# mlefkir/Pioran.jl

Measured on AMD Instinct MI355X. Metric: logpdf evals/sec (batched) at N=1e4, J=20; max |Δlogℒ| vs reference, higher is better.
Workload: dtype f64; 1 GPU; N=10000 irregular series, SHO-20 (J=20 celerite terms, R=40 active rows), batch=4096 draws per GPU, shared (c,d), per-draw mu/nu; inputs HBM-resident; N=10000, J=20, R_active=40, batch_per_gpu=4096, global_batch=4096, kernel_config=tile, parallelism=batch-sharded x1, all-gather of logL

## Files before the change

pioran.jl_amd/csrc/celerite_tile.hip:

```cpp
#include "common.h"
#include "window_common.h"

#ifndef PIORAN_TSTAMP
#define PIORAN_TSTAMP(i) __builtin_amdgcn_sched_barrier(0)
#define PIORAN_TSTAMP_DECL
#define PIORAN_TSTAMP_FLUSH
#endif
#ifndef PIORAN_ASTAMP2
#define PIORAN_ASTAMP2(i) __builtin_amdgcn_sched_barrier(0)
#define PIORAN_ASTAMP2_DECL
#define PIORAN_ASTAMP2_FLUSH
#endif

namespace {

#ifndef PIORAN_TILE_FWD_NOWAIT
#define PIORAN_TILE_FWD_NOWAIT 1
#endif
#if PIORAN_TILE_FWD_NOWAIT
#define PIORAN_TILE_FWD_ORDER() asm volatile("" ::: "memory")
#else
#define PIORAN_TILE_FWD_ORDER() asm volatile("s_waitcnt lgkmcnt(0)" ::: "memory")
#endif
#ifndef PIORAN_TILE_ADJ_RAGFIX
#define PIORAN_TILE_ADJ_RAGFIX 1
#endif
#ifndef PIORAN_TILE_RAGFIX4
#define PIORAN_TILE_RAGFIX4 1
#endif
#ifndef PIORAN_TILE_QUADALL
#define PIORAN_TILE_QUADALL 1
#endif
#ifndef PIORAN_TILE_RAGFIX
#define PIORAN_TILE_RAGFIX 1
#endif
#ifndef PIORAN_TILE_YSFIX
#define PIORAN_TILE_YSFIX 1
#endif
#ifndef PIORAN_TILE_BIG_VHA
#define PIORAN_TILE_BIG_VHA 1
#endif
#ifndef PIORAN_TILE_BIG_CKP
#define PIORAN_TILE_BIG_CKP 1
#endif
#ifndef PIORAN_TILE_VHA
#define PIORAN_TILE_VHA 1
#endif
constexpr int kTileMaxTerms = 64;
constexpr int kTileWaves = 4;
#define PIORAN_LDS_ORDER() asm volatile("" ::: "memory")
template <int NB, bool CD = false>
constexpr int tile_adj_waves() { return NB <= 3 ? 4 : (CD ? 2 : 3); }

typedef unsigned int tile_u32x2 __attribute__((ext_vector_type(2)));
__device__ __forceinline__ double tile_bload(__amdgpu_buffer_rsrc_t rs, int voff, int soff)
{
    const tile_u32x2 v = __builtin_amdgcn_raw_buffer_load_b64(rs, voff, soff, 0);
    return __hiloint2double((int)v.y, (int)v.x);
}

template <int NB>
struct TileWave {
    double scr[16 * 18];
    double2 albe[16 * NB];
    double ck[16 * NB + 16];
    double ys[16];
    double up[NB > 1 ? NB * (NB - 1) / 2 : 1][16 * 18];
};

constexpr int kPairWin = 5;
template <int JQ>
__global__ void __launch_bounds__(256) tile_pairs_mfma_kernel(const ScanParams p, const double* __restrict__ btab, int64_t rsb, int64_t tsp, double* __restrict__ out)
{
    const int J = p.J;
    const int64_t NW = (p.N + KW - 1) / KW;
    const int lane = threadIdx.x & 63, w = threadIdx.x >> 6, li = lane & 15, lk = lane >> 4;
    const int64_t b0 = ((int64_t)blockIdx.y * 4 + w) * 16;
    if (b0 >= p.B) return;
    const int64_t draw = b0 + li < p.B ? b0 + li : p.B - 1;
    double aop[JQ], bop[JQ];
    int toff[JQ];
#pragma unroll
    for (int q = 0; q < JQ; ++q) {
        const int t = 4 * q + lk;
        aop[q] = t < J ? p.A[draw * J + t] : 0.0;
        bop[q] = t < J ? p.Bc[draw * J + t] : 0.0;
        toff[q] = (t < J ? t : J - 1) * 128 + 4 * (li & 3) + (li >> 2);
    }
    const bool live = b0 + li < p.B;
    double* orow = out + (b0 + li) * NW * 128 + 4 * lk;
    const int64_t k0 = (int64_t)blockIdx.x * kPairWin, k1 = k0 + kPairWin < NW ? k0 + kPairWin : NW;
    for (int64_t k = k0; k < k1; ++k) {
        const double2* E = reinterpret_cast<const double2*>(btab + k * rsb + tsp);
#pragma unroll 2
        for (int pt = 0; pt < 8; ++pt) {
            double2 e[JQ];
#pragma unroll
            for (int q = 0; q < JQ; ++q) e[q] = E[toff[q] + 16 * pt];
            d4 acc = {0.0, 0.0, 0.0, 0.0};
#pragma unroll
            for (int q = 0; q < JQ; ++q) {
                acc = __builtin_amdgcn_mfma_f64_16x16x4f64(e[q].x, aop[q], acc, 0, 0, 0);
                acc = __builtin_amdgcn_mfma_f64_16x16x4f64(e[q].y, bop[q], acc, 0, 0, 0);
            }
            if (live) *reinterpret_cast<d4*>(orow + k * 128 + 16 * pt) = acc;
        }
    }
}

template <typename... Args>
static inline bool launch_pairs_mfma(const ScanParams& p, hipStream_t stream, Args... args)
{
    const int64_t NW = (p.N + KW - 1) / KW;
    if ((p.B + 63) / 64 > 65535 || p.J > kTileMaxTerms) return false;
    const dim3 gr((unsigned)((NW + kPairWin - 1) / kPairWin), (unsigned)((p.B + 63) / 64));
    const int jq = (p.J + 3) / 4;
    if (jq <= 5) hipLaunchKernelGGL(tile_pairs_mfma_kernel<5>, gr, dim3(256), 0, stream, p, args...);
    else if (jq <= 10) hipLaunchKernelGGL(tile_pairs_mfma_kernel<10>, gr, dim3(256), 0, stream, p, args...);
    else if (jq <= 16) hipLaunchKernelGGL(tile_pairs_mfma_kernel<16>, gr, dim3(256), 0, stream, p, args...);
    else return false;
    return true;
}

template <int NB, int KL = 4, bool ST = false>
__global__ void __launch_bounds__(64 * kTileWaves, NB <= 4 ? 2 : 1) celerite_tile_kernel(const ScanParams p, const double* __restrict__ btab,
                                                                                          const double* __restrict__ pairs)
// ... 29 lines not shown
            const int rm = p.rowmap[r];
            const int term = rm & 0xfffff;
            a = Ab_[term];
            bb = ((rm >> 30) & 1) ? -Bb_[term] : Bb_[term];
        }
        sw.albe[r] = double2{a, bb};
    }
    constexpr int NU = NB * (NB - 1) / 2;
    for (int i = lane; i < (NU > 0 ? NU : 1) * 16 * 18; i += 64) (&sw.up[0][0])[i] = 0.0;
    asm volatile("s_waitcnt lgkmcnt(0)" ::: "memory");

    constexpr int NT = NB * (NB + 1) / 2;
    auto tix = [](int I, int Jc) constexpr { return I * (I + 1) / 2 + Jc; };
    auto uix = [](int I, int Jc) constexpr { return I * (I - 1) / 2 + Jc; };
    d4 T[NT];
#pragma unroll
    for (int i = 0; i < NT; ++i) T[i] = d4{0.0, 0.0, 0.0, 0.0};
    double Uf[NB][4];

    double cvn[4], cxn[4];
    auto live_k = [](int I, int ks) constexpr { return I < NB - 1 || ks < KL; };
    auto fetch_u = [&](int64_t k, int I) __attribute__((always_inline)) {
        const int so = (int)k * rsb8;
#pragma unroll
        for (int ks = 0; ks < 4; ++ks) {
            if (!live_k(I, ks)) continue;
            cvn[ks] = tile_bload(rs_tab, lane8, so + (I * 4 + ks) * 512);
            cxn[ks] = tile_bload(rs_tab, lane8, so + (NB * 256 + (I * 4 + ks) * 64) * 8);
        }
    };
    auto form_u = [&](int I) __attribute__((always_inline)) {
        if (I == NB - 1 && KL == 0) return;
        double2 cf[4];
#pragma unroll
        for (int ks = 0; ks < 4; ++ks)
            if (live_k(I, ks)) cf[ks] = sw.albe[16 * I + 4 * ks + q];
        asm volatile("s_waitcnt lgkmcnt(0)" ::: "memory");
#pragma unroll
        for (int ks = 0; ks < 4; ++ks)
            if (live_k(I, ks)) Uf[I][ks] = fma(cf[ks].x, cvn[ks], cf[ks].y * cxn[ks]);
    };
    constexpr int NCK = (16 * NB + 16 + 63) / 64;
    double ckpre[NCK];
    auto fetch_ck = [&](int64_t k) __attribute__((always_inline)) {
        const int so = (int)k * rsb8 + 3 * NB * 256 * 8;
#pragma unroll
        for (int i = 0; i < NCK; ++i) ckpre[i] = tile_bload(rs_tab, lane8, so + 512 * i);
    };
    int pidx[4];
#pragma unroll
    for (int g = 0; g < 4; ++g) {
        const int r = 4 * g + q, hi = r > c16 ? r : c16, lo = r > c16 ? c16 : r;
        pidx[g] = 8 * (r == c16 ? 127 : hi * (hi - 1) / 2 + lo);
    }
    const int gd = (c16 - q) >> 2;
    const bool on_diag = ((c16 - q) & 3) == 0;
    double apre[4];
    auto fetch_A = [&](int64_t k) __attribute__((always_inline)) {
#pragma unroll
        for (int g = 0; g < 4; ++g) apre[g] = tile_bload(rs_pw, pidx[g], (int)k * 1024);
    };
    const bool has_series = p.Y != nullptr;
    double ypre = 0.0, spre = 0.0;
    auto fetch_series = [&](int64_t k) __attribute__((always_inline)) {
        if (has_series) {
            int64_t n = k * KW + c16;
            n = n < N ? n : N - 1;
            ypre = p.Y[b * N + n];
            spre = p.S2[b * N + n];
        }
    };
    fetch_A(0);
    fetch_ck(0);
    fetch_series(0);
#pragma unroll
    for (int I = 0; I < NB; ++I) {
        fetch_u(0, I);
        form_u(I);
    }
    double mu_sel[NB];
#pragma unroll
    for (int Jc = 0; Jc < NB; ++Jc) mu_sel[Jc] = (Jc == Jy && c16 == ry) ? mu : 0.0;
    const int64_t k_ragged = (N % KW) ? NW - 1 : NW;
    double quad = 0.0;
#if PIORAN_TILE_QUADALL
    double quadb[NB];
#pragma unroll
    for (int I = 0; I < NB; ++I) quadb[I] = 0.0;
#endif
    double Pm = 1.0;
    int Pe = 0;
    bool nonpd = false;

    PIORAN_TSTAMP_DECL
    for (int64_t k = 0; k < NW; ++k) {
        PIORAN_TSTAMP(0);
        const int wso = (int)k * rsb8;
        const bool more = k + 1 < NW;
#pragma unroll
        for (int i = 0; i < NCK; ++i)
            if (lane + 64 * i < 16 * NB + 16) sw.ck[lane + 64 * i] = ckpre[i];
        if (has_series) {
            asm volatile("s_waitcnt lgkmcnt(0)" ::: "memory");
            if (lane < 16) { sw.ys[lane] = ypre; sw.ck[16 * NB + lane] = spre; }
        }
        if (more) { fetch_ck(k + 1); fetch_series(k + 1); }
        if constexpr (ST) {
            d4* gtk = reinterpret_cast<d4*>(p.gw + ((b * NW + k) * NT) * 256);
#pragma unroll
            for (int i = 0; i < NT; ++i) gtk[i * 64 + lane] = T[i];
        }
        constexpr bool VHA = PIORAN_TILE_VHA && (NB <= 3 || (PIORAN_TILE_BIG_VHA && NB >= 5));
        [[maybe_unused]] double vha[VHA ? NB : 1][4];
        if constexpr (VHA) {
#pragma unroll
            for (int I = 0; I < NB; ++I)
#pragma unroll
                for (int g = 0; g < 4; ++g) vha[I][g] = tile_bload(rs_tab, lane8, wso + (2 * NB * 256 + (I * 4 + g) * 64) * 8);
#if PIORAN_TILE_RAGFIX
            if (k == k_ragged) {
#pragma unroll
                for (int I = 0; I < NB; ++I)
#pragma unroll
                    for (int g = 0; g < 4; ++g)
                        if (k * KW + 4 * g + q >= N) vha[I][g] = mu_sel[I];
            }
#endif
        }
        d4 x[NB];
#pragma unroll
        for (int Jc = 0; Jc < NB; ++Jc) {
            d4 acc = {0.0, 0.0, 0.0, 0.0};
#pragma unroll
            for (int I = 0; I < Jc; ++I) {
                double bt[4];
#pragma unroll
                for (int ks = 0; ks < 4; ++ks) bt[ks] = sw.up[uix(Jc, I)][c16 * 18 + 4 * ks + q];
#pragma unroll
                for (int ks = 0; ks < 4; ++ks) acc = __builtin_amdgcn_mfma_f64_16x16x4f64(Uf[I][ks], bt[ks], acc, 0, 0, 0);
            }
#pragma unroll
            for (int I = Jc; I < NB; ++I)
#pragma unroll
                for (int ks = 0; ks < 4; ++ks)
                    if (live_k(I, ks)) acc = __builtin_amdgcn_mfma_f64_16x16x4f64(Uf[I][ks], T[tix(I, Jc)][ks], acc, 0, 0, 0);
            x[Jc] = acc;
        }
        PIORAN_TSTAMP(1);
        d4 G = {0.0, 0.0, 0.0, 0.0};
        double vh[4];
        if constexpr (!VHA) {
#pragma unroll
            for (int g = 0; g < 4; ++g) vh[g] = tile_bload(rs_tab, lane8, wso + (2 * NB * 256 + g * 64) * 8);
        }
        double ysv[4] = {0.0, 0.0, 0.0, 0.0};
        if (has_series) {
#pragma unroll
            for (int g = 0; g < 4; ++g) ysv[g] = sw.ys[4 * g + q];
        }
#pragma unroll
        for (int Jc = 0; Jc < NB; ++Jc) {
            const bool gk = Jc < NB - 1 || KL > 0;
            if (gk) {
#pragma unroll
                for (int g = 0; g < 4; ++g) sw.scr[(4 * g + q) * 18 + c16] = x[Jc][g];
            }
            PIORAN_TILE_FWD_ORDER();
            double mb[4];
#pragma unroll
            for (int ks = 0; ks < 4; ++ks)
                if (live_k(Jc, ks)) mb[ks] = sw.scr[c16 * 18 + 4 * ks + q];
            const double ckc = sw.ck[16 * Jc + c16];
            asm volatile("s_waitcnt lgkmcnt(0)" ::: "memory");
#pragma unroll
            for (int ks = 0; ks < 4; ++ks)
                if (live_k(Jc, ks)) G = __builtin_amdgcn_mfma_f64_16x16x4f64(Uf[Jc][ks], mb[ks], G, 0, 0, 0);
#pragma unroll
            for (int g = 0; g < 4; ++g) {
                double v;
                if constexpr (VHA) v = vha[Jc][g]; else v = vh[g];
#if !PIORAN_TILE_YSFIX
                if (has_series && Jc == Jy && c16 == ry) v = ysv[g];
#endif
                v -= mu_sel[Jc];
#if PIORAN_TILE_RAGFIX && !PIORAN_TILE_RAGFIX4
                if constexpr (!VHA)
#endif
#if !PIORAN_TILE_RAGFIX4
                if (k == k_ragged && k * KW + 4 * g + q >= N) v = 0.0;
#endif
                x[Jc][g] = fma(-ckc, x[Jc][g], v);
                asm volatile("" : "+v"(x[Jc][g]));
            }
            if constexpr (!VHA) {
                if (Jc + 1 < NB) {
#pragma unroll
                    for (int g = 0; g < 4; ++g) vh[g] = tile_bload(rs_tab, lane8, wso + (2 * NB * 256 + ((Jc + 1) * 4 + g) * 64) * 8);
                }
            }
            __builtin_amdgcn_sched_barrier(0);
        }
#if PIORAN_TILE_RAGFIX4
        if constexpr (!VHA) {
            if (k == k_ragged) {
#pragma unroll
                for (int Jc = 0; Jc < NB; ++Jc)
#pragma unroll
                    for (int g = 0; g < 4; ++g) {
                        const double vt = tile_bload(rs_tab, lane8, wso + (2 * NB * 256 + (Jc * 4 + g) * 64) * 8);
                        if (k * KW + 4 * g + q >= N) x[Jc][g] -= vt - mu_sel[Jc];
                    }
            }
        }
#endif
#if PIORAN_TILE_YSFIX
        if (has_series) {
            static_for<0, NB>([&](auto Jcc) __attribute__((always_inline)) {
                constexpr int Jc = decltype(Jcc)::value;
                if (Jc == Jy) {
#pragma unroll
                    for (int g = 0; g < 4; ++g) {
                        double vt;
                        if constexpr (VHA) vt = vha[Jc][g]; else vt = tile_bload(rs_tab, lane8, wso + (2 * NB * 256 + (Jc * 4 + g) * 64) * 8);
                        const bool pad = k == k_ragged && k * KW + 4 * g + q >= N;
                        if (c16 == ry && !pad) x[Jc][g] += ysv[g] - vt;
                    }
                }
            });
        }
#endif
        PIORAN_TSTAMP(2);
        PIORAN_TSTAMP(3);
        {
            const double s2n = sw.ck[16 * NB + c16];
            const double dg = k * KW + c16 < N ? suma + (has_nu ? nu * s2n : s2n) : 1.0;
#pragma unroll
            for (int g = 0; g < 4; ++g) sw.scr[(4 * g + q) * 16 + c16] = ((on_diag && g == gd) ? dg : apre[g]) - G[g];
        }
        if (k + 1 < NW) fetch_A(k + 1);
        PIORAN_TILE_FWD_ORDER();
        double m[16];
#pragma unroll
        for (int j = 0; j < 16; ++j) m[j] = sw.scr[j * 16 + c16];
        asm volatile("s_waitcnt lgkmcnt(0)" ::: "memory");
        PIORAN_TSTAMP(4);
        __builtin_amdgcn_s_setprio(2);
        double mult = ldl_first_mult(m, c16);
        static_for<0, 16>([&](auto Pc) __attribute__((always_inline)) { ldl_step<decltype(Pc)::value>(m, mult, c16); });
        __builtin_amdgcn_s_setprio(0);
        PIORAN_TSTAMP(5);
        if (q == 0) {
            double2* dst = reinterpret_cast<double2*>(sw.scr + c16 * 18);
#pragma unroll
            for (int j = 0; j < 16; j += 2) dst[j / 2] = double2{m[j], m[j + 1]};
        }
        PIORAN_TILE_FWD_ORDER();
        double li[4], idv[4];
#pragma unroll
        for (int ks = 0; ks < 4; ++ks) {
            const int kk = 4 * ks + q;
            const double lv = sw.scr[kk * 18 + c16];
            idv[ks] = recip_f64(sw.scr[kk * 18 + kk]);
            li[ks] = kk < c16 ? lv * idv[ks] : (kk == c16 ? 1.0 : 0.0);
        }
        {
            const double dj = sw.scr[c16 * 18 + c16];
            nonpd |= !(dj > 0.0);
            Pm *= (k == 0 && c16 == 0) ? dj : fabs(dj);
            int ex;
            Pm = frexp(Pm, &ex);
            Pe += ex;
        }
        asm volatile("s_waitcnt lgkmcnt(0)" ::: "memory");
        PIORAN_TSTAMP(6);
        if (more) fetch_u(k + 1, 0);
        __builtin_amdgcn_sched_barrier(0);
        d4 yt[NB];
#pragma unroll
        for (int Jc = 0; Jc < NB; ++Jc) {
            d4 a = {0.0, 0.0, 0.0, 0.0};
#pragma unroll
            for (int ks = 0; ks < 4; ++ks) a = __builtin_amdgcn_mfma_f64_16x16x4f64(li[ks], x[Jc][ks], a, 0, 0, 0);
            yt[Jc] = a;
        }
        PIORAN_TSTAMP(7);
        constexpr bool CKP = NB <= 3 || (PIORAN_TILE_BIG_CKP && NB >= 5);
        [[maybe_unused]] double ckrow[CKP ? NB : 1][4], ckcol[CKP ? NB : 1];
        if constexpr (CKP) {
#pragma unroll
            for (int I = 0; I < NB; ++I) {
#pragma unroll
                for (int g = 0; g < 4; ++g) ckrow[I][g] = sw.ck[16 * I + 4 * g + q];
                ckcol[I] = sw.ck[16 * I + c16];
            }
        }
        auto ck_row = [&](int I, int g) __attribute__((always_inline)) -> double { if constexpr (CKP) return ckrow[I][g]; else return sw.ck[16 * I + 4 * g + q]; };
#pragma unroll
        for (int Jc = 0; Jc < NB; ++Jc) {
            if (more) {
                form_u(Jc);
                if (Jc + 1 < NB) fetch_u(k + 1, Jc + 1);
            }
            double ysc[4];
            double ckc;
            if constexpr (CKP) ckc = ckcol[Jc]; else ckc = sw.ck[16 * Jc + c16];
#pragma unroll
            for (int g = 0; g < 4; ++g) {
                ysc[g] = yt[Jc][g] * idv[g];
#if PIORAN_TILE_QUADALL
                quadb[Jc] = fma(yt[Jc][g], ysc[g], quadb[Jc]);
#else
                if (Jc == Jy) quad = fma(yt[Jc][g], ysc[g], quad);
#endif
            }
#pragma unroll
            for (int I = Jc; I < NB; ++I) {
#pragma unroll
                for (int g = 0; g < 4; ++g) T[tix(I, Jc)][g] *= ck_row(I, g) * ckc;
#pragma unroll
                for (int ks = 0; ks < 4; ++ks) T[tix(I, Jc)] = __builtin_amdgcn_mfma_f64_16x16x4f64(yt[I][ks], ysc[ks], T[tix(I, Jc)], 0, 0, 0);
                if (Jc < I) {
#pragma unroll
                    for (int g = 0; g < 4; ++g) sw.up[uix(I, Jc)][(4 * g + q) * 18 + c16] = T[tix(I, Jc)][g];
                }
            }
            __builtin_amdgcn_sched_barrier(0);
        }
        PIORAN_TSTAMP(8);
        PIORAN_TILE_FWD_ORDER();
    }

    PIORAN_TSTAMP_FLUSH
    asm volatile("s_waitcnt lgkmcnt(0)" ::: "memory");
#if PIORAN_TILE_QUADALL
#pragma unroll
    for (int I = 0; I < NB; ++I)
        if (I == Jy) quad = quadb[I];
// ... 1010 lines not shown
```

pioran.jl_amd/csrc/ldl_steps.inc:

```
template <int P> __device__ __forceinline__ void ldl_step_fused(double (&m)[16], double& mult, int c16);
template <> __device__ __forceinline__ void ldl_step_fused<0>(double (&m)[16], double& mult, int c16)
{
    double dn, r0, e, t0, pq, mn;
    asm volatile("v_fmac_f64_dpp %[m1], %[m1], %[t] row_newbcast:0 row_mask:0xf bank_mask:0xf\n\t"
                 "s_nop 1\n\tv_mov_b64_dpp %[dn], %[m1] row_newbcast:1 row_mask:0xf bank_mask:0xf\n\t"
                 "v_rcp_f64 %[r0], %[dn]\n\t"
                 "v_fmac_f64_dpp %[m2], %[m2], %[t] row_newbcast:0 row_mask:0xf bank_mask:0xf\n\t"
                 "v_fmac_f64_dpp %[m3], %[m3], %[t] row_newbcast:0 row_mask:0xf bank_mask:0xf\n\t"
                 "v_fmac_f64_dpp %[m4], %[m4], %[t] row_newbcast:0 row_mask:0xf bank_mask:0xf\n\t"
                 "v_fmac_f64_dpp %[m5], %[m5], %[t] row_newbcast:0 row_mask:0xf bank_mask:0xf\n\t"
                 "v_fma_f64 %[e], -%[r0], %[dn], 1.0\n\tv_mul_f64 %[t0], -%[m1], %[r0]\n\t"
                 "v_fmac_f64_dpp %[m6], %[m6], %[t] row_newbcast:0 row_mask:0xf bank_mask:0xf\n\t"
                 "v_fmac_f64_dpp %[m7], %[m7], %[t] row_newbcast:0 row_mask:0xf bank_mask:0xf\n\t"
                 "v_fmac_f64_dpp %[m8], %[m8], %[t] row_newbcast:0 row_mask:0xf bank_mask:0xf\n\t"
                 "v_fmac_f64_dpp %[m9], %[m9], %[t] row_newbcast:0 row_mask:0xf bank_mask:0xf\n\t"
                 "v_fma_f64 %[pq], %[e], %[e], %[e]\n\t"
                 "v_fmac_f64_dpp %[m10], %[m10], %[t] row_newbcast:0 row_mask:0xf bank_mask:0xf\n\t"
                 "v_fmac_f64_dpp %[m11], %[m11], %[t] row_newbcast:0 row_mask:0xf bank_mask:0xf\n\t"
                 "v_fmac_f64_dpp %[m12], %[m12], %[t] row_newbcast:0 row_mask:0xf bank_mask:0xf\n\t"
                 "v_fmac_f64_dpp %[m13], %[m13], %[t] row_newbcast:0 row_mask:0xf bank_mask:0xf\n\t"
                 "v_fmac_f64_dpp %[m14], %[m14], %[t] row_newbcast:0 row_mask:0xf bank_mask:0xf\n\t"
                 "v_fmac_f64_dpp %[m15], %[m15], %[t] row_newbcast:0 row_mask:0xf bank_mask:0xf\n\t"
                 "v_fma_f64 %[mn], %[t0], %[pq], %[t0]"
                 : [m1] "+v"(m[1]), [m2] "+v"(m[2]), [m3] "+v"(m[3]), [m4] "+v"(m[4]), [m5] "+v"(m[5]), [m6] "+v"(m[6]), [m7] "+v"(m[7]), [m8] "+v"(m[8]), [m9] "+v"(m[9]), [m10] "+v"(m[10]), [m11] "+v"(m[11]), [m12] "+v"(m[12]), [m13] "+v"(m[13]), [m14] "+v"(m[14]), [m15] "+v"(m[15]), [dn] "=&v"(dn), [r0] "=&v"(r0), [e] "=&v"(e), [t0] "=&v"(t0), [pq] "=&v"(pq), [mn] "=&v"(mn)
// ... 195 lines not shown
                 "v_fma_f64 %[pq], %[e], %[e], %[e]\n\t"
                 "v_fma_f64 %[mn], %[t0], %[pq], %[t0]"
                 : [m10] "+v"(m[10]), [m11] "+v"(m[11]), [m12] "+v"(m[12]), [m13] "+v"(m[13]), [m14] "+v"(m[14]), [m15] "+v"(m[15]), [dn] "=&v"(dn), [r0] "=&v"(r0), [e] "=&v"(e), [t0] "=&v"(t0), [pq] "=&v"(pq), [mn] "=&v"(mn)
                 : [t] "v"(mult));
    mult = c16 == 10 ? -2.0 : mn;
}
template <> __device__ __forceinline__ void ldl_step_fused<10>(double (&m)[16], double& mult, int c16)
{
    double dn, r0, e, t0, pq, mn;
    asm volatile("v_fmac_f64_dpp %[m11], %[m11], %[t] row_newbcast:10 row_mask:0xf bank_mask:0xf\n\t"
                 "s_nop 1\n\tv_mov_b64_dpp %[dn], %[m11] row_newbcast:11 row_mask:0xf bank_mask:0xf\n\t"
                 "v_rcp_f64 %[r0], %[dn]\n\t"
                 "v_fmac_f64_dpp %[m12], %[m12], %[t] row_newbcast:10 row_mask:0xf bank_mask:0xf\n\t"
                 "v_fmac_f64_dpp %[m13], %[m13], %[t] row_newbcast:10 row_mask:0xf bank_mask:0xf\n\t"
                 "v_fmac_f64_dpp %[m14], %[m14], %[t] row_newbcast:10 row_mask:0xf bank_mask:0xf\n\t"
                 "v_fmac_f64_dpp %[m15], %[m15], %[t] row_newbcast:10 row_mask:0xf bank_mask:0xf\n\t"
                 "v_fma_f64 %[e], -%[r0], %[dn], 1.0\n\tv_mul_f64 %[t0], -%[m11], %[r0]\n\t"
                 "v_fma_f64 %[pq], %[e], %[e], %[e]\n\t"
                 "v_fma_f64 %[mn], %[t0], %[pq], %[t0]"
                 : [m11] "+v"(m[11]), [m12] "+v"(m[12]), [m13] "+v"(m[13]), [m14] "+v"(m[14]), [m15] "+v"(m[15]), [dn] "=&v"(dn), [r0] "=&v"(r0), [e] "=&v"(e), [t0] "=&v"(t0), [pq] "=&v"(pq), [mn] "=&v"(mn)
                 : [t] "v"(mult));
    mult = c16 == 11 ? -2.0 : mn;
}
template <> __device__ __forceinline__ void ldl_step_fused<11>(double (&m)[16], double& mult, int c16)
{
    double dn, r0, e, t0, pq, mn;
    asm volatile("v_fmac_f64_dpp %[m12], %[m12], %[t] row_newbcast:11 row_mask:0xf bank_mask:0xf\n\t"
                 "s_nop 1\n\tv_mov_b64_dpp %[dn], %[m12] row_newbcast:12 row_mask:0xf bank_mask:0xf\n\t"
                 "v_rcp_f64 %[r0], %[dn]\n\t"
                 "v_fmac_f64_dpp %[m13], %[m13], %[t] row_newbcast:11 row_mask:0xf bank_mask:0xf\n\t"
                 "v_fmac_f64_dpp %[m14], %[m14], %[t] row_newbcast:11 row_mask:0xf bank_mask:0xf\n\t"
                 "v_fmac_f64_dpp %[m15], %[m15], %[t] row_newbcast:11 row_mask:0xf bank_mask:0xf\n\t"
                 "v_fma_f64 %[e], -%[r0], %[dn], 1.0\n\tv_mul_f64 %[t0], -%[m12], %[r0]\n\t"
                 "v_fma_f64 %[pq], %[e], %[e], %[e]\n\t"
                 "v_fma_f64 %[mn], %[t0], %[pq], %[t0]"
                 : [m12] "+v"(m[12]), [m13] "+v"(m[13]), [m14] "+v"(m[14]), [m15] "+v"(m[15]), [dn] "=&v"(dn), [r0] "=&v"(r0), [e] "=&v"(e), [t0] "=&v"(t0), [pq] "=&v"(pq), [mn] "=&v"(mn)
                 : [t] "v"(mult));
    mult = c16 == 12 ? -2.0 : mn;
}
template <> __device__ __forceinline__ void ldl_step_fused<12>(double (&m)[16], double& mult, int c16)
{
    double dn, r0, e, t0, pq, mn;
    asm volatile("v_fmac_f64_dpp %[m13], %[m13], %[t] row_newbcast:12 row_mask:0xf bank_mask:0xf\n\t"
                 "s_nop 1\n\tv_mov_b64_dpp %[dn], %[m13] row_newbcast:13 row_mask:0xf bank_mask:0xf\n\t"
                 "v_rcp_f64 %[r0], %[dn]\n\t"
                 "v_fmac_f64_dpp %[m14], %[m14], %[t] row_newbcast:12 row_mask:0xf bank_mask:0xf\n\t"
                 "v_fmac_f64_dpp %[m15], %[m15], %[t] row_newbcast:12 row_mask:0xf bank_mask:0xf\n\t"
                 "v_fma_f64 %[e], -%[r0], %[dn], 1.0\n\tv_mul_f64 %[t0], -%[m13], %[r0]\n\t"
                 "v_fma_f64 %[pq], %[e], %[e], %[e]\n\t"
                 "v_fma_f64 %[mn], %[t0], %[pq], %[t0]"
                 : [m13] "+v"(m[13]), [m14] "+v"(m[14]), [m15] "+v"(m[15]), [dn] "=&v"(dn), [r0] "=&v"(r0), [e] "=&v"(e), [t0] "=&v"(t0), [pq] "=&v"(pq), [mn] "=&v"(mn)
                 : [t] "v"(mult));
    mult = c16 == 13 ? -2.0 : mn;
}
template <> __device__ __forceinline__ void ldl_step_fused<13>(double (&m)[16], double& mult, int c16)
{
    double dn, r0, e, t0, pq, mn;
    asm volatile("v_fmac_f64_dpp %[m14], %[m14], %[t] row_newbcast:13 row_mask:0xf bank_mask:0xf\n\t"
                 "s_nop 1\n\tv_mov_b64_dpp %[dn], %[m14] row_newbcast:14 row_mask:0xf bank_mask:0xf\n\t"
                 "v_rcp_f64 %[r0], %[dn]\n\t"
                 "v_fmac_f64_dpp %[m15], %[m15], %[t] row_newbcast:13 row_mask:0xf bank_mask:0xf\n\t"
                 "v_fma_f64 %[e], -%[r0], %[dn], 1.0\n\tv_mul_f64 %[t0], -%[m14], %[r0]\n\t"
                 "v_fma_f64 %[pq], %[e], %[e], %[e]\n\t"
                 "v_fma_f64 %[mn], %[t0], %[pq], %[t0]"
                 : [m14] "+v"(m[14]), [m15] "+v"(m[15]), [dn] "=&v"(dn), [r0] "=&v"(r0), [e] "=&v"(e), [t0] "=&v"(t0), [pq] "=&v"(pq), [mn] "=&v"(mn)
                 : [t] "v"(mult));
    mult = c16 == 14 ? -2.0 : mn;
}
template <> __device__ __forceinline__ void ldl_step_fused<14>(double (&m)[16], double& mult, int c16)
{
    double dn, r0, e, t0, pq, mn;
    asm volatile("v_fmac_f64_dpp %[m15], %[m15], %[t] row_newbcast:14 row_mask:0xf bank_mask:0xf\n\t"
                 "s_nop 1\n\tv_mov_b64_dpp %[dn], %[m15] row_newbcast:15 row_mask:0xf bank_mask:0xf\n\t"
                 "v_rcp_f64 %[r0], %[dn]\n\t"
                 "s_nop 0\n\t"
                 "v_fma_f64 %[e], -%[r0], %[dn], 1.0\n\tv_mul_f64 %[t0], -%[m15], %[r0]\n\t"
                 "v_fma_f64 %[pq], %[e], %[e], %[e]\n\t"
                 "v_fma_f64 %[mn], %[t0], %[pq], %[t0]"
                 : [m15] "+v"(m[15]), [dn] "=&v"(dn), [r0] "=&v"(r0), [e] "=&v"(e), [t0] "=&v"(t0), [pq] "=&v"(pq), [mn] "=&v"(mn)
                 : [t] "v"(mult));
    mult = c16 == 15 ? -2.0 : mn;
}
template <> __device__ __forceinline__ void ldl_step_fused<15>(double (&)[16], double&, int) {}
```

pioran.jl_amd/csrc/window_common.h:

```cpp
#pragma once
#include "common.h"

#include <cmath>
#include <type_traits>

namespace {

typedef double d4 __attribute__((ext_vector_type(4)));

template <int I>
using ic = std::integral_constant<int, I>;
template <int B, int E, class F>
__device__ __forceinline__ void static_for(F&& f)
{
    if constexpr (B < E) {
        f(ic<B>{});
        static_for<B + 1, E>(f);
    }
}

__device__ __forceinline__ double recip_f64(double x)
{
    double r = __builtin_amdgcn_rcp(x);
    r = fma(fma(-x, r, 1.0), r, r);
    r = fma(fma(-x, r, 1.0), r, r);
    return r;
}

constexpr int KW = 16;

__host__ __device__ inline int64_t block_rec_doubles(int NB, int J) { return ((3 * (int64_t)NB * 256 + 16 * NB + 16 + 127) & ~(int64_t)127) + (int64_t)J * 256; }

__device__ __forceinline__ void blk_rcp(double& r, double d) { asm volatile("v_rcp_f64 %0, %1" : "=v"(r) : "v"(d)); }
__device__ __forceinline__ void blk_e_t0(double& e, double& t0, double r0, double d, double mrow)
{
    asm volatile("s_nop 0\n\tv_fma_f64 %0, -%2, %3, 1.0\n\tv_mul_f64 %1, -%4, %2" : "=&v"(e), "=&v"(t0) : "v"(r0), "v"(d), "v"(mrow));
}
__device__ __forceinline__ void blk_poly(double& pq, double e) { asm volatile("v_fma_f64 %0, %1, %1, %1" : "=v"(pq) : "v"(e)); }
__device__ __forceinline__ void blk_mult(double& mu_, double t0, double pq) { asm volatile("v_fma_f64 %0, %1, %2, %1" : "=v"(mu_) : "v"(t0), "v"(pq)); }
#include "ldl_steps.inc"
template <int P>
__device__ __forceinline__ void ldl_step(double (&m)[16], double& mult, int c16)
{
    ldl_step_fused<P>(m, mult, c16);
}
__device__ __forceinline__ double ldl_first_mult(double (&m)[16], int c16)
{
    double d0, r0, e, t0, pq, mn;
    asm volatile("s_nop 1\n\tv_mov_b64_dpp %0, %1 row_newbcast:0 row_mask:0xf bank_mask:0xf" : "=v"(d0) : "v"(m[0]));
    asm volatile("s_nop 0");
    blk_rcp(r0, d0);
    blk_e_t0(e, t0, r0, d0, m[0]);
    blk_poly(pq, e);
    blk_mult(mn, t0, pq);
    return c16 == 0 ? -2.0 : mn;
}

__host__ __device__ inline int block_tile_doubles(int NB) { return (3 * NB * 256 + 16 * NB + 16 + 127) & ~127; }

__device__ __forceinline__ void dma_pieces(const double* gsrc, double* ldst, int npieces, int w, int nwaves, int lane)
{
    for (int c = w; c < npieces; c += nwaves)
        __builtin_amdgcn_global_load_lds((const __attribute__((address_space(1))) void*)(gsrc + c * 128 + lane * 2),
                                         (__attribute__((address_space(3))) void*)(ldst + c * 128), 16, 0, 0);
}
__device__ __forceinline__ void dma_pieces_asm(const double* gsrc, double* ldst, int npieces, int w, int nwaves, int lane)
{
    const unsigned lbase = (unsigned)(uintptr_t)(__attribute__((address_space(3))) void*)ldst;
    for (int c = w; c < npieces; c += nwaves) {
        const double* g = gsrc + c * 128 + lane * 2;
        const unsigned l = __builtin_amdgcn_readfirstlane(lbase + (unsigned)c * 1024u);
        unsigned m0_save;
        asm volatile("s_mov_b32 %0, m0\n\ts_mov_b32 m0, %2\n\ts_nop 0\n\tglobal_load_lds_dwordx4 %1, off\n\ts_mov_b32 m0, %0"
                     : "=&s"(m0_save)
                     : "v"(g), "s"(l)
                     : "memory");
    }
}
#define PIORAN_BLK_BARRIER() asm volatile("s_waitcnt lgkmcnt(0)\n\ts_barrier" ::: "memory")
#define PIORAN_BLK_BARRIER_DMA() asm volatile("s_waitcnt vmcnt(0) lgkmcnt(0)\n\ts_barrier" ::: "memory")

}
```

Measured before the change: 440,800 evals/s.

## Split 16x16 diagonal-block LDL across four lane groups with LDS pivot exchange

Before, each lane loaded a full 16-element column of the diagonal block from LDS and ran the whole 16-step DPP LDL elimination on it. The new path has each of the four q-groups keep only 4 rows in registers. At every step the pivot row is passed through an LDS write/read pair, so each lane issues about a quarter of the FMAs. The aim is to cut the LDS transpose round trip and the per-lane FMA count on the serial critical path. In exchange, every pivot step now carries an LDS latency and an s_waitcnt, and all of it is hand-written inline asm with row masks that could be wrong.

```diff
diff --git a/pioran.jl_amd/csrc/celerite_tile.hip b/pioran.jl_amd/csrc/celerite_tile.hip
--- a/pioran.jl_amd/csrc/celerite_tile.hip
+++ b/pioran.jl_amd/csrc/celerite_tile.hip
@@ -42,6 +42,15 @@
 #endif
 #ifndef PIORAN_TILE_BIG_CKP
 #define PIORAN_TILE_BIG_CKP 1
+#endif
+#ifndef PIORAN_TILE_LDL_SPLIT
+#define PIORAN_TILE_LDL_SPLIT 1
+#endif
+#ifndef PIORAN_TILE_LDL_SPLIT_MAXNB
+#define PIORAN_TILE_LDL_SPLIT_MAXNB 4
+#endif
+#ifndef PIORAN_TILE_LDL_PRIO
+#define PIORAN_TILE_LDL_PRIO 2
 #endif
 #ifndef PIORAN_TILE_VHA
 #define PIORAN_TILE_VHA 1
@@ -237,6 +246,9 @@
 #pragma unroll
     for (int Jc = 0; Jc < NB; ++Jc) mu_sel[Jc] = (Jc == Jy && c16 == ry) ? mu : 0.0;
     const int64_t k_ragged = (N % KW) ? NW - 1 : NW;
+    constexpr bool LDL_SPLIT = PIORAN_TILE_LDL_SPLIT && !ST && NB <= PIORAN_TILE_LDL_SPLIT_MAXNB;
+    [[maybe_unused]] const unsigned ldl_ra = (unsigned)(uintptr_t)(__attribute__((address_space(3))) void*)sw.scr + 8u * (unsigned)c16;
+    [[maybe_unused]] const unsigned ldl_wa = ldl_ra + 128u * (unsigned)q;
     double quad = 0.0;
 #if PIORAN_TILE_QUADALL
     double quadb[NB];
@@ -386,28 +398,41 @@
 #endif
         PIORAN_TSTAMP(2);
         PIORAN_TSTAMP(3);
-        {
-            const double s2n = sw.ck[16 * NB + c16];
-            const double dg = k * KW + c16 < N ? suma + (has_nu ? nu * s2n : s2n) : 1.0;
+        const double s2n = sw.ck[16 * NB + c16];
+        const double dg = k * KW + c16 < N ? suma + (has_nu ? nu * s2n : s2n) : 1.0;
+        if constexpr (LDL_SPLIT) {
+            double m[4];
+#pragma unroll
+            for (int g = 0; g < 4; ++g) m[g] = ((on_diag && g == gd) ? dg : apre[g]) - G[g];
+            if (k + 1 < NW) fetch_A(k + 1);
+            PIORAN_TSTAMP(4);
+            __builtin_amdgcn_s_setprio(PIORAN_TILE_LDL_PRIO);
+            double mult = ldl4_first_mult(m, c16, ldl_wa, ldl_ra);
+            static_for<0, 15>([&](auto Pc) __attribute__((always_inline)) { ldl4_step<decltype(Pc)::value>(m, mult, c16, ldl_wa, ldl_ra); });
+            __builtin_amdgcn_s_setprio(0);
+            PIORAN_TSTAMP(5);
+#pragma unroll
+            for (int g = 0; g < 4; ++g) sw.scr[c16 * 18 + 4 * g + q] = m[g];
+        } else {
 #pragma unroll
             for (int g = 0; g < 4; ++g) sw.scr[(4 * g + q) * 16 + c16] = ((on_diag && g == gd) ? dg : apre[g]) - G[g];
-        }
-        if (k + 1 < NW) fetch_A(k + 1);
-        PIORAN_TILE_FWD_ORDER();
-        double m[16];
-#pragma unroll
-        for (int j = 0; j < 16; ++j) m[j] = sw.scr[j * 16 + c16];
-        asm volatile("s_waitcnt lgkmcnt(0)" ::: "memory");
-        PIORAN_TSTAMP(4);
-        __builtin_amdgcn_s_setprio(2);
-        double mult = ldl_first_mult(m, c16);
-        static_for<0, 16>([&](auto Pc) __attribute__((always_inline)) { ldl_step<decltype(Pc)::value>(m, mult, c16); });
-        __builtin_amdgcn_s_setprio(0);
-        PIORAN_TSTAMP(5);
-        if (q == 0) {
-            double2* dst = reinterpret_cast<double2*>(sw.scr + c16 * 18);
-#pragma unroll
-            for (int j = 0; j < 16; j += 2) dst[j / 2] = double2{m[j], m[j + 1]};
+            if (k + 1 < NW) fetch_A(k + 1);
+            PIORAN_TILE_FWD_ORDER();
+            double m[16];
+#pragma unroll
+            for (int j = 0; j < 16; ++j) m[j] = sw.scr[j * 16 + c16];
+            asm volatile("s_waitcnt lgkmcnt(0)" ::: "memory");
+            PIORAN_TSTAMP(4);
+            __builtin_amdgcn_s_setprio(2);
+            double mult = ldl_first_mult(m, c16);
+            static_for<0, 16>([&](auto Pc) __attribute__((always_inline)) { ldl_step<decltype(Pc)::value>(m, mult, c16); });
+            __builtin_amdgcn_s_setprio(0);
+            PIORAN_TSTAMP(5);
+            if (q == 0) {
+                double2* dst = reinterpret_cast<double2*>(sw.scr + c16 * 18);
+#pragma unroll
+                for (int j = 0; j < 16; j += 2) dst[j / 2] = double2{m[j], m[j + 1]};
+            }
         }
         PIORAN_TILE_FWD_ORDER();
         double li[4], idv[4];
diff --git a/pioran.jl_amd/csrc/ldl_steps.inc b/pioran.jl_amd/csrc/ldl_steps.inc
--- a/pioran.jl_amd/csrc/ldl_steps.inc
+++ b/pioran.jl_amd/csrc/ldl_steps.inc
@@ -301,3 +301,241 @@
     mult = c16 == 15 ? -2.0 : mn;
 }
 template <> __device__ __forceinline__ void ldl_step_fused<15>(double (&)[16], double&, int) {}
+template <int P> __device__ __forceinline__ void ldl4_step_fused(double (&m)[4], double& mult, int c16, unsigned wa, unsigned ra);
+template <> __device__ __forceinline__ void ldl4_step_fused<0>(double (&m)[4], double& mult, int c16, unsigned wa, unsigned ra)
+{
+    double mr, dn, r0, e, t0, pq, mn;
+    asm volatile("v_fmac_f64_dpp %[m0], %[m0], %[t] row_newbcast:0 row_mask:0xe bank_mask:0xf\n\t"
+                 "ds_write_b64 %[wa], %[m0]\n\tds_read_b64 %[mr], %[ra] offset:128\n\t"
+                 "v_fmac_f64_dpp %[m1], %[m1], %[t] row_newbcast:0 row_mask:0xf bank_mask:0xf\n\t"
+                 "v_fmac_f64_dpp %[m2], %[m2], %[t] row_newbcast:0 row_mask:0xf bank_mask:0xf\n\t"
+                 "v_fmac_f64_dpp %[m3], %[m3], %[t] row_newbcast:0 row_mask:0xf bank_mask:0xf\n\t"
+                 "s_waitcnt lgkmcnt(0)\n\tv_mov_b64_dpp %[dn], %[mr] row_newbcast:1 row_mask:0xf bank_mask:0xf\n\t"
+                 "v_rcp_f64 %[r0], %[dn]\n\ts_nop 0\n\t"
+                 "v_fma_f64 %[e], -%[r0], %[dn], 1.0\n\tv_mul_f64 %[t0], -%[mr], %[r0]\n\t"
+                 "v_fma_f64 %[pq], %[e], %[e], %[e]\n\t"
+                 "v_fma_f64 %[mn], %[t0], %[pq], %[t0]"
+                 : [m0] "+v"(m[0]), [m1] "+v"(m[1]), [m2] "+v"(m[2]), [m3] "+v"(m[3]), [mr] "=&v"(mr), [dn] "=&v"(dn), [r0] "=&v"(r0), [e] "=&v"(e), [t0] "=&v"(t0), [pq] "=&v"(pq), [mn] "=&v"(mn)
+                 : [t] "v"(mult), [wa] "v"(wa), [ra] "v"(ra)
+                 : "memory");
+    mult = c16 == 1 ? -2.0 : mn;
+}
+template <> __device__ __forceinline__ void ldl4_step_fused<1>(double (&m)[4], double& mult, int c16, unsigned wa, unsigned ra)
+{
+    double mr, dn, r0, e, t0, pq, mn;
+    asm volatile("v_fmac_f64_dpp %[m0], %[m0], %[t] row_newbcast:1 row_mask:0xc bank_mask:0xf\n\t"
+                 "ds_write_b64 %[wa], %[m0]\n\tds_read_b64 %[mr], %[ra] offset:256\n\t"
+                 "v_fmac_f64_dpp %[m1], %[m1], %[t] row_newbcast:1 row_mask:0xf bank_mask:0xf\n\t"
+                 "v_fmac_f64_dpp %[m2], %[m2], %[t] row_newbcast:1 row_mask:0xf bank_mask:0xf\n\t"
+                 "v_fmac_f64_dpp %[m3], %[m3], %[t] row_newbcast:1 row_mask:0xf bank_mask:0xf\n\t"
+                 "s_waitcnt lgkmcnt(0)\n\tv_mov_b64_dpp %[dn], %[mr] row_newbcast:2 row_mask:0xf bank_mask:0xf\n\t"
+                 "v_rcp_f64 %[r0], %[dn]\n\ts_nop 0\n\t"
+                 "v_fma_f64 %[e], -%[r0], %[dn], 1.0\n\tv_mul_f64 %[t0], -%[mr], %[r0]\n\t"
+                 "v_fma_f64 %[pq], %[e], %[e], %[e]\n\t"
+                 "v_fma_f64 %[mn], %[t0], %[pq], %[t0]"
+                 : [m0] "+v"(m[0]), [m1] "+v"(m[1]), [m2] "+v"(m[2]), [m3] "+v"(m[3]), [mr] "=&v"(mr), [dn] "=&v"(dn), [r0] "=&v"(r0), [e] "=&v"(e), [t0] "=&v"(t0), [pq] "=&v"(pq), [mn] "=&v"(mn)
+                 : [t] "v"(mult), [wa] "v"(wa), [ra] "v"(ra)
+                 : "memory");
+    mult = c16 == 2 ? -2.0 : mn;
+}
+template <> __device__ __forceinline__ void ldl4_step_fused<2>(double (&m)[4], double& mult, int c16, unsigned wa, unsigned ra)
+{
+    double mr, dn, r0, e, t0, pq, mn;
+    asm volatile("v_fmac_f64_dpp %[m0], %[m0], %[t] row_newbcast:2 row_mask:0x8 bank_mask:0xf\n\t"
+                 "ds_write_b64 %[wa], %[m0]\n\tds_read_b64 %[mr], %[ra] offset:384\n\t"
+                 "v_fmac_f64_dpp %[m1], %[m1], %[t] row_newbcast:2 row_mask:0xf bank_mask:0xf\n\t"
+                 "v_fmac_f64_dpp %[m2], %[m2], %[t] row_newbcast:2 row_mask:0xf bank_mask:0xf\n\t"
+                 "v_fmac_f64_dpp %[m3], %[m3], %[t] row_newbcast:2 row_mask:0xf bank_mask:0xf\n\t"
+                 "s_waitcnt lgkmcnt(0)\n\tv_mov_b64_dpp %[dn], %[mr] row_newbcast:3 row_mask:0xf bank_mask:0xf\n\t"
+                 "v_rcp_f64 %[r0], %[dn]\n\ts_nop 0\n\t"
+                 "v_fma_f64 %[e], -%[r0], %[dn], 1.0\n\tv_mul_f64 %[t0], -%[mr], %[r0]\n\t"
+                 "v_fma_f64 %[pq], %[e], %[e], %[e]\n\t"
+                 "v_fma_f64 %[mn], %[t0], %[pq], %[t0]"
+                 : [m0] "+v"(m[0]), [m1] "+v"(m[1]), [m2] "+v"(m[2]), [m3] "+v"(m[3]), [mr] "=&v"(mr), [dn] "=&v"(dn), [r0] "=&v"(r0), [e] "=&v"(e), [t0] "=&v"(t0), [pq] "=&v"(pq), [mn] "=&v"(mn)
+                 : [t] "v"(mult), [wa] "v"(wa), [ra] "v"(ra)
+                 : "memory");
+    mult = c16 == 3 ? -2.0 : mn;
+}
+template <> __device__ __forceinline__ void ldl4_step_fused<3>(double (&m)[4], double& mult, int c16, unsigned wa, unsigned ra)
+{
+    double mr, dn, r0, e, t0, pq, mn;
+    asm volatile("v_fmac_f64_dpp %[m1], %[m1], %[t] row_newbcast:3 row_mask:0xf bank_mask:0xf\n\t"
+                 "ds_write_b64 %[wa], %[m1]\n\tds_read_b64 %[mr], %[ra] offset:0\n\t"
+                 "v_fmac_f64_dpp %[m2], %[m2], %[t] row_newbcast:3 row_mask:0xf bank_mask:0xf\n\t"
+                 "v_fmac_f64_dpp %[m3], %[m3], %[t] row_newbcast:3 row_mask:0xf bank_mask:0xf\n\t"
+                 "s_waitcnt lgkmcnt(0)\n\tv_mov_b64_dpp %[dn], %[mr] row_newbcast:4 row_mask:0xf bank_mask:0xf\n\t"
+                 "v_rcp_f64 %[r0], %[dn]\n\ts_nop 0\n\t"
+                 "v_fma_f64 %[e], -%[r0], %[dn], 1.0\n\tv_mul_f64 %[t0], -%[mr], %[r0]\n\t"
+                 "v_fma_f64 %[pq], %[e], %[e], %[e]\n\t"
+                 "v_fma_f64 %[mn], %[t0], %[pq], %[t0]"
+                 : [m1] "+v"(m[1]), [m2] "+v"(m[2]), [m3] "+v"(m[3]), [mr] "=&v"(mr), [dn] "=&v"(dn), [r0] "=&v"(r0), [e] "=&v"(e), [t0] "=&v"(t0), [pq] "=&v"(pq), [mn] "=&v"(mn)
+                 : [t] "v"(mult), [wa] "v"(wa), [ra] "v"(ra)
+                 : "memory");
+    mult = c16 == 4 ? -2.0 : mn;
+}
+template <> __device__ __forceinline__ void ldl4_step_fused<4>(double (&m)[4], double& mult, int c16, unsigned wa, unsigned ra)
+{
+    double mr, dn, r0, e, t0, pq, mn;
+    asm volatile("v_fmac_f64_dpp %[m1], %[m1], %[t] row_newbcast:4 row_mask:0xe bank_mask:0xf\n\t"
+                 "ds_write_b64 %[wa], %[m1]\n\tds_read_b64 %[mr], %[ra] offset:128\n\t"
+                 "v_fmac_f64_dpp %[m2], %[m2], %[t] row_newbcast:4 row_mask:0xf bank_mask:0xf\n\t"
+                 "v_fmac_f64_dpp %[m3], %[m3], %[t] row_newbcast:4 row_mask:0xf bank_mask:0xf\n\t"
+                 "s_waitcnt lgkmcnt(0)\n\tv_mov_b64_dpp %[dn], %[mr] row_newbcast:5 row_mask:0xf bank_mask:0xf\n\t"
+                 "v_rcp_f64 %[r0], %[dn]\n\ts_nop 0\n\t"
+                 "v_fma_f64 %[e], -%[r0], %[dn], 1.0\n\tv_mul_f64 %[t0], -%[mr], %[r0]\n\t"
+                 "v_fma_f64 %[pq], %[e], %[e], %[e]\n\t"
+                 "v_fma_f64 %[mn], %[t0], %[pq], %[t0]"
+                 : [m1] "+v"(m[1]), [m2] "+v"(m[2]), [m3] "+v"(m[3]), [mr] "=&v"(mr), [dn] "=&v"(dn), [r0] "=&v"(r0), [e] "=&v"(e), [t0] "=&v"(t0), [pq] "=&v"(pq), [mn] "=&v"(mn)
+                 : [t] "v"(mult), [wa] "v"(wa), [ra] "v"(ra)
+                 : "memory");
+    mult = c16 == 5 ? -2.0 : mn;
+}
+template <> __device__ __forceinline__ void ldl4_step_fused<5>(double (&m)[4], double& mult, int c16, unsigned wa, unsigned ra)
+{
+    double mr, dn, r0, e, t0, pq, mn;
+    asm volatile("v_fmac_f64_dpp %[m1], %[m1], %[t] row_newbcast:5 row_mask:0xc bank_mask:0xf\n\t"
+                 "ds_write_b64 %[wa], %[m1]\n\tds_read_b64 %[mr], %[ra] offset:256\n\t"
+                 "v_fmac_f64_dpp %[m2], %[m2], %[t] row_newbcast:5 row_mask:0xf bank_mask:0xf\n\t"
+                 "v_fmac_f64_dpp %[m3], %[m3], %[t] row_newbcast:5 row_mask:0xf bank_mask:0xf\n\t"
+                 "s_waitcnt lgkmcnt(0)\n\tv_mov_b64_dpp %[dn], %[mr] row_newbcast:6 row_mask:0xf bank_mask:0xf\n\t"
+                 "v_rcp_f64 %[r0], %[dn]\n\ts_nop 0\n\t"
+                 "v_fma_f64 %[e], -%[r0], %[dn], 1.0\n\tv_mul_f64 %[t0], -%[mr], %[r0]\n\t"
+                 "v_fma_f64 %[pq], %[e], %[e], %[e]\n\t"
+                 "v_fma_f64 %[mn], %[t0], %[pq], %[t0]"
+                 : [m1] "+v"(m[1]), [m2] "+v"(m[2]), [m3] "+v"(m[3]), [mr] "=&v"(mr), [dn] "=&v"(dn), [r0] "=&v"(r0), [e] "=&v"(e), [t0] "=&v"(t0), [pq] "=&v"(pq), [mn] "=&v"(mn)
+                 : [t] "v"(mult), [wa] "v"(wa), [ra] "v"(ra)
+                 : "memory");
+    mult = c16 == 6 ? -2.0 : mn;
+}
+template <> __device__ __forceinline__ void ldl4_step_fused<6>(double (&m)[4], double& mult, int c16, unsigned wa, unsigned ra)
+{
+    double mr, dn, r0, e, t0, pq, mn;
+    asm volatile("v_fmac_f64_dpp %[m1], %[m1], %[t] row_newbcast:6 row_mask:0x8 bank_mask:0xf\n\t"
+                 "ds_write_b64 %[wa], %[m1]\n\tds_read_b64 %[mr], %[ra] offset:384\n\t"
+                 "v_fmac_f64_dpp %[m2], %[m2], %[t] row_newbcast:6 row_mask:0xf bank_mask:0xf\n\t"
+                 "v_fmac_f64_dpp %[m3], %[m3], %[t] row_newbcast:6 row_mask:0xf bank_mask:0xf\n\t"
+                 "s_waitcnt lgkmcnt(0)\n\tv_mov_b64_dpp %[dn], %[mr] row_newbcast:7 row_mask:0xf bank_mask:0xf\n\t"
+                 "v_rcp_f64 %[r0], %[dn]\n\ts_nop 0\n\t"
+                 "v_fma_f64 %[e], -%[r0], %[dn], 1.0\n\tv_mul_f64 %[t0], -%[mr], %[r0]\n\t"
+                 "v_fma_f64 %[pq], %[e], %[e], %[e]\n\t"
+                 "v_fma_f64 %[mn], %[t0], %[pq], %[t0]"
+                 : [m1] "+v"(m[1]), [m2] "+v"(m[2]), [m3] "+v"(m[3]), [mr] "=&v"(mr), [dn] "=&v"(dn), [r0] "=&v"(r0), [e] "=&v"(e), [t0] "=&v"(t0), [pq] "=&v"(pq), [mn] "=&v"(mn)
+                 : [t] "v"(mult), [wa] "v"(wa), [ra] "v"(ra)
+                 : "memory");
+    mult = c16 == 7 ? -2.0 : mn;
+}
+template <> __device__ __forceinline__ void ldl4_step_fused<7>(double (&m)[4], double& mult, int c16, unsigned wa, unsigned ra)
+{
+    double mr, dn, r0, e, t0, pq, mn;
+    asm volatile("v_fmac_f64_dpp %[m2], %[m2], %[t] row_newbcast:7 row_mask:0xf bank_mask:0xf\n\t"
+                 "ds_write_b64 %[wa], %[m2]\n\tds_read_b64 %[mr], %[ra] offset:0\n\t"
+                 "v_fmac_f64_dpp %[m3], %[m3], %[t] row_newbcast:7 row_mask:0xf bank_mask:0xf\n\t"
+                 "s_waitcnt lgkmcnt(0)\n\tv_mov_b64_dpp %[dn], %[mr] row_newbcast:8 row_mask:0xf bank_mask:0xf\n\t"
+                 "v_rcp_f64 %[r0], %[dn]\n\ts_nop 0\n\t"
+                 "v_fma_f64 %[e], -%[r0], %[dn], 1.0\n\tv_mul_f64 %[t0], -%[mr], %[r0]\n\t"
+                 "v_fma_f64 %[pq], %[e], %[e], %[e]\n\t"
+                 "v_fma_f64 %[mn], %[t0], %[pq], %[t0]"
+                 : [m2] "+v"(m[2]), [m3] "+v"(m[3]), [mr] "=&v"(mr), [dn] "=&v"(dn), [r0] "=&v"(r0), [e] "=&v"(e), [t0] "=&v"(t0), [pq] "=&v"(pq), [mn] "=&v"(mn)
+                 : [t] "v"(mult), [wa] "v"(wa), [ra] "v"(ra)
+                 : "memory");
+    mult = c16 == 8 ? -2.0 : mn;
+}
+template <> __device__ __forceinline__ void ldl4_step_fused<8>(double (&m)[4], double& mult, int c16, unsigned wa, unsigned ra)
+{
+    double mr, dn, r0, e, t0, pq, mn;
+    asm volatile("v_fmac_f64_dpp %[m2], %[m2], %[t] row_newbcast:8 row_mask:0xe bank_mask:0xf\n\t"
+                 "ds_write_b64 %[wa], %[m2]\n\tds_read_b64 %[mr], %[ra] offset:128\n\t"
+                 "v_fmac_f64_dpp %[m3], %[m3], %[t] row_newbcast:8 row_mask:0xf bank_mask:0xf\n\t"
+                 "s_waitcnt lgkmcnt(0)\n\tv_mov_b64_dpp %[dn], %[mr] row_newbcast:9 row_mask:0xf bank_mask:0xf\n\t"
+                 "v_rcp_f64 %[r0], %[dn]\n\ts_nop 0\n\t"
+                 "v_fma_f64 %[e], -%[r0], %[dn], 1.0\n\tv_mul_f64 %[t0], -%[mr], %[r0]\n\t"
+                 "v_fma_f64 %[pq], %[e], %[e], %[e]\n\t"
+                 "v_fma_f64 %[mn], %[t0], %[pq], %[t0]"
+                 : [m2] "+v"(m[2]), [m3] "+v"(m[3]), [mr] "=&v"(mr), [dn] "=&v"(dn), [r0] "=&v"(r0), [e] "=&v"(e), [t0] "=&v"(t0), [pq] "=&v"(pq), [mn] "=&v"(mn)
+                 : [t] "v"(mult), [wa] "v"(wa), [ra] "v"(ra)
+                 : "memory");
+    mult = c16 == 9 ? -2.0 : mn;
+}
+template <> __device__ __forceinline__ void ldl4_step_fused<9>(double (&m)[4], double& mult, int c16, unsigned wa, unsigned ra)
+{
+    double mr, dn, r0, e, t0, pq, mn;
+    asm volatile("v_fmac_f64_dpp %[m2], %[m2], %[t] row_newbcast:9 row_mask:0xc bank_mask:0xf\n\t"
+                 "ds_write_b64 %[wa], %[m2]\n\tds_read_b64 %[mr], %[ra] offset:256\n\t"
+                 "v_fmac_f64_dpp %[m3], %[m3], %[t] row_newbcast:9 row_mask:0xf bank_mask:0xf\n\t"
+                 "s_waitcnt lgkmcnt(0)\n\tv_mov_b64_dpp %[dn], %[mr] row_newbcast:10 row_mask:0xf bank_mask:0xf\n\t"
+                 "v_rcp_f64 %[r0], %[dn]\n\ts_nop 0\n\t"
+                 "v_fma_f64 %[e], -%[r0], %[dn], 1.0\n\tv_mul_f64 %[t0], -%[mr], %[r0]\n\t"
+                 "v_fma_f64 %[pq], %[e], %[e], %[e]\n\t"
+                 "v_fma_f64 %[mn], %[t0], %[pq], %[t0]"
+                 : [m2] "+v"(m[2]), [m3] "+v"(m[3]), [mr] "=&v"(mr), [dn] "=&v"(dn), [r0] "=&v"(r0), [e] "=&v"(e), [t0] "=&v"(t0), [pq] "=&v"(pq), [mn] "=&v"(mn)
+                 : [t] "v"(mult), [wa] "v"(wa), [ra] "v"(ra)
+                 : "memory");
+    mult = c16 == 10 ? -2.0 : mn;
+}
+template <> __device__ __forceinline__ void ldl4_step_fused<10>(double (&m)[4], double& mult, int c16, unsigned wa, unsigned ra)
+{
+    double mr, dn, r0, e, t0, pq, mn;
+    asm volatile("v_fmac_f64_dpp %[m2], %[m2], %[t] row_newbcast:10 row_mask:0x8 bank_mask:0xf\n\t"
+                 "ds_write_b64 %[wa], %[m2]\n\tds_read_b64 %[mr], %[ra] offset:384\n\t"
+                 "v_fmac_f64_dpp %[m3], %[m3], %[t] row_newbcast:10 row_mask:0xf bank_mask:0xf\n\t"
+                 "s_waitcnt lgkmcnt(0)\n\tv_mov_b64_dpp %[dn], %[mr] row_newbcast:11 row_mask:0xf bank_mask:0xf\n\t"
+                 "v_rcp_f64 %[r0], %[dn]\n\ts_nop 0\n\t"
+                 "v_fma_f64 %[e], -%[r0], %[dn], 1.0\n\tv_mul_f64 %[t0], -%[mr], %[r0]\n\t"
+                 "v_fma_f64 %[pq], %[e], %[e], %[e]\n\t"
+                 "v_fma_f64 %[mn], %[t0], %[pq], %[t0]"
+                 : [m2] "+v"(m[2]), [m3] "+v"(m[3]), [mr] "=&v"(mr), [dn] "=&v"(dn), [r0] "=&v"(r0), [e] "=&v"(e), [t0] "=&v"(t0), [pq] "=&v"(pq), [mn] "=&v"(mn)
+                 : [t] "v"(mult), [wa] "v"(wa), [ra] "v"(ra)
+                 : "memory");
+    mult = c16 == 11 ? -2.0 : mn;
+}
+template <> __device__ __forceinline__ void ldl4_step_fused<11>(double (&m)[4], double& mult, int c16, unsigned wa, unsigned ra)
+{
+    double mr, dn, r0, e, t0, pq, mn;
+    asm volatile("v_fmac_f64_dpp %[m3], %[m3], %[t] row_newbcast:11 row_mask:0xf bank_mask:0xf\n\t"
+                 "ds_write_b64 %[wa], %[m3]\n\tds_read_b64 %[mr], %[ra] offset:0\n\t"
+                 "s_waitcnt lgkmcnt(0)\n\tv_mov_b64_dpp %[dn], %[mr] row_newbcast:12 row_mask:0xf bank_mask:0xf\n\t"
+                 "v_rcp_f64 %[r0], %[dn]\n\ts_nop 0\n\t"
+                 "v_fma_f64 %[e], -%[r0], %[dn], 1.0\n\tv_mul_f64 %[t0], -%[mr], %[r0]\n\t"
+                 "v_fma_f64 %[pq], %[e], %[e], %[e]\n\t"
+                 "v_fma_f64 %[mn], %[t0], %[pq], %[t0]"
+                 : [m3] "+v"(m[3]), [mr] "=&v"(mr), [dn] "=&v"(dn), [r0] "=&v"(r0), [e] "=&v"(e), [t0] "=&v"(t0), [pq] "=&v"(pq), [mn] "=&v"(mn)
+                 : [t] "v"(mult), [wa] "v"(wa), [ra] "v"(ra)
+                 : "memory");
+    mult = c16 == 12 ? -2.0 : mn;
+}
+template <> __device__ __forceinline__ void ldl4_step_fused<12>(double (&m)[4], double& mult, int c16, unsigned wa, unsigned ra)
+{
+    double mr, dn, r0, e, t0, pq, mn;
+    asm volatile("v_fmac_f64_dpp %[m3], %[m3], %[t] row_newbcast:12 row_mask:0xe bank_mask:0xf\n\t"
+                 "ds_write_b64 %[wa], %[m3]\n\tds_read_b64 %[mr], %[ra] offset:128\n\t"
+                 "s_waitcnt lgkmcnt(0)\n\tv_mov_b64_dpp %[dn], %[mr] row_newbcast:13 row_mask:0xf bank_mask:0xf\n\t"
+                 "v_rcp_f64 %[r0], %[dn]\n\ts_nop 0\n\t"
+                 "v_fma_f64 %[e], -%[r0], %[dn], 1.0\n\tv_mul_f64 %[t0], -%[mr], %[r0]\n\t"
+                 "v_fma_f64 %[pq], %[e], %[e], %[e]\n\t"
+                 "v_fma_f64 %[mn], %[t0], %[pq], %[t0]"
+                 : [m3] "+v"(m[3]), [mr] "=&v"(mr), [dn] "=&v"(dn), [r0] "=&v"(r0), [e] "=&v"(e), [t0] "=&v"(t0), [pq] "=&v"(pq), [mn] "=&v"(mn)
+                 : [t] "v"(mult), [wa] "v"(wa), [ra] "v"(ra)
+                 : "memory");
+    mult = c16 == 13 ? -2.0 : mn;
+}
+template <> __device__ __forceinline__ void ldl4_step_fused<13>(double (&m)[4], double& mult, int c16, unsigned wa, unsigned ra)
+{
+    double mr, dn, r0, e, t0, pq, mn;
+    asm volatile("v_fmac_f64_dpp %[m3], %[m3], %[t] row_newbcast:13 row_mask:0xc bank_mask:0xf\n\t"
+                 "ds_write_b64 %[wa], %[m3]\n\tds_read_b64 %[mr], %[ra] offset:256\n\t"
+                 "s_waitcnt lgkmcnt(0)\n\tv_mov_b64_dpp %[dn], %[mr] row_newbcast:14 row_mask:0xf bank_mask:0xf\n\t"
+                 "v_rcp_f64 %[r0], %[dn]\n\ts_nop 0\n\t"
+                 "v_fma_f64 %[e], -%[r0], %[dn], 1.0\n\tv_mul_f64 %[t0], -%[mr], %[r0]\n\t"
+                 "v_fma_f64 %[pq], %[e], %[e], %[e]\n\t"
+                 "v_fma_f64 %[mn], %[t0], %[pq], %[t0]"
+                 : [m3] "+v"(m[3]), [mr] "=&v"(mr), [dn] "=&v"(dn), [r0] "=&v"(r0), [e] "=&v"(e), [t0] "=&v"(t0), [pq] "=&v"(pq), [mn] "=&v"(mn)
+                 : [t] "v"(mult), [wa] "v"(wa), [ra] "v"(ra)
+                 : "memory");
+    mult = c16 == 14 ? -2.0 : mn;
+}
+template <> __device__ __forceinline__ void ldl4_step_fused<14>(double (&m)[4], double& mult, int, unsigned, unsigned)
+{
+    asm volatile("v_fmac_f64_dpp %[m3], %[m3], %[t] row_newbcast:14 row_mask:0x8 bank_mask:0xf"
+                 : [m3] "+v"(m[3])
+                 : [t] "v"(mult));
+}
diff --git a/pioran.jl_amd/csrc/window_common.h b/pioran.jl_amd/csrc/window_common.h
--- a/pioran.jl_amd/csrc/window_common.h
+++ b/pioran.jl_amd/csrc/window_common.h
@@ -56,6 +56,26 @@
     return c16 == 0 ? -2.0 : mn;
 }
 
+template <int P>
+__device__ __forceinline__ void ldl4_step(double (&m)[4], double& mult, int c16, unsigned wa, unsigned ra)
+{
+    ldl4_step_fused<P>(m, mult, c16, wa, ra);
+}
+__device__ __forceinline__ double ldl4_first_mult(double (&m)[4], int c16, unsigned wa, unsigned ra)
+{
+    double mr, d0, r0, e, t0, pq, mn;
+    asm volatile("ds_write_b64 %[wa], %[m0]\n\tds_read_b64 %[mr], %[ra]\n\t"
+                 "s_waitcnt lgkmcnt(0)\n\tv_mov_b64_dpp %[dn], %[mr] row_newbcast:0 row_mask:0xf bank_mask:0xf\n\t"
+                 "v_rcp_f64 %[r0], %[dn]\n\ts_nop 0\n\t"
+                 "v_fma_f64 %[e], -%[r0], %[dn], 1.0\n\tv_mul_f64 %[t0], -%[mr], %[r0]\n\t"
+                 "v_fma_f64 %[pq], %[e], %[e], %[e]\n\t"
+                 "v_fma_f64 %[mn], %[t0], %[pq], %[t0]"
+                 : [mr] "=&v"(mr), [dn] "=&v"(d0), [r0] "=&v"(r0), [e] "=&v"(e), [t0] "=&v"(t0), [pq] "=&v"(pq), [mn] "=&v"(mn)
+                 : [m0] "v"(m[0]), [wa] "v"(wa), [ra] "v"(ra)
+                 : "memory");
+    return c16 == 0 ? -2.0 : mn;
+}
+
 __host__ __device__ inline int block_tile_doubles(int NB) { return (3 * NB * 256 + 16 * NB + 16 + 127) & ~127; }
 
 __device__ __forceinline__ void dma_pieces(const double* gsrc, double* ldst, int npieces, int w, int nwaves, int lane)
```

After: 444,800 evals/s (median of 6 runs). About the same (+0.9%).
